# caoql98/LKGD

Measured on AMD Instinct MI355X. Metric: denoised frames/sec (14f x 576x1024, 25-step Euler), higher is better.
Workload: dtype f16; 1 GPU; SVD 14 frames x 576x1024, 25 Euler steps, CFG 1.0->3.0, single clip, vanilla pipeline_stable_video_diffusion_trans loop (configs[1]); unet=random-init SVD shapes (320,640,1280,1280), heads (5,10,20,20), 1.52 B params, parallelism=single GPU

## Files before the change

### lkgd_amd/csrc/gemm.hip

```cpp
#include "gemm_common.h"

#define BM 128
#define BN 128
#define STAGE_BYTES (2 * BM * BK * 2)
#define GEMM_LDS (2 * STAGE_BYTES)

__global__ __launch_bounds__(256, 2) void lkgd_gemm_kernel(const lkgd_gemm_desc p, int tiles_m, int tiles_n, int ksplit,
                                                           int per, float* ws) {
  extern __shared__ __attribute__((aligned(16))) char smem[];
  const int t = threadIdx.x;
  const int lane = t & 63;
  const int w = t >> 6;
  const int wr = w >> 1, wc = w & 1;

  const int nwg = tiles_m * tiles_n;
  const int bid = xcd_remap(blockIdx.x, nwg);
  const int tm = bid / tiles_n, tn = bid - tm * tiles_n;
  const int m0 = tm * BM, n0 = tn * BN;

  const int srow = t >> 3;
  const int schunk = (t & 7) ^ ((t >> 4) & 7);
  AGather<4> ag;
  const half_t* brow[4];
#pragma unroll
  for (int i = 0; i < 4; ++i) {
    ag.row[i] = a_row(p, m0 + srow + 32 * i);
    int n = n0 + srow + 32 * i;
    brow[i] = n < p.N ? (const half_t*)p.w + (long long)n * p.K + schunk * 8 : nullptr;
  }
  const int nk_all = p.K / BK;
  const int kb = ksplit > 1 ? (int)blockIdx.y * per : 0;
  const int ke = ksplit > 1 ? (kb + per < nk_all ? kb + per : nk_all) : nk_all;
  a_segment<4>(p, ag, kb * BK, schunk);

  auto stage = [&](int buf, int kt) {
    char* sa = smem + buf * STAGE_BYTES;
    char* sb = sa + BM * BK * 2;
    const int k0 = kt * BK;
    if (k0 >= ag.seg_end) a_segment<4>(p, ag, k0, schunk);
#pragma unroll
    for (int i = 0; i < 4; ++i) glds16(a_chunk<4>(ag, i, k0), sa + (w * 64 + 256 * i) * 16);
#pragma unroll
    for (int i = 0; i < 4; ++i)
      glds16(brow[i] ? brow[i] + k0 : (const half_t*)p.zeros, sb + (w * 64 + 256 * i) * 16);
  };

  float16_t acc[2][2];
#pragma unroll
  for (int i = 0; i < 2; ++i)
#pragma unroll
    for (int j = 0; j < 2; ++j)
#pragma unroll
      for (int r = 0; r < 16; ++r) acc[i][j][r] = 0.f;

  const int h = lane >> 5;
  int a_off[2], b_off[2], a_sw[2], b_sw[2];
#pragma unroll
  for (int i = 0; i < 2; ++i) {
    int ra = wr * 64 + i * 32 + (lane & 31);
    int rb = wc * 64 + i * 32 + (lane & 31);
    a_off[i] = ra * 128; a_sw[i] = (ra >> 1) & 7;
    b_off[i] = BM * BK * 2 + rb * 128; b_sw[i] = (rb >> 1) & 7;
  }

  stage(0, kb);
  asm volatile("s_waitcnt vmcnt(0)" ::: "memory");
  __syncthreads();
  for (int kt = kb; kt < ke; ++kt) {
    const int cur = (kt - kb) & 1;
    if (kt + 1 < ke) stage(cur ^ 1, kt + 1);
    const char* sbase = smem + cur * STAGE_BYTES;
#pragma unroll
    for (int ks = 0; ks < 4; ++ks) {
      half8_t af[2], bf[2];
#pragma unroll
      for (int i = 0; i < 2; ++i) {
        af[i] = *(const half8_t*)(sbase + a_off[i] + (((ks * 2 + h) ^ a_sw[i]) << 4));
        bf[i] = *(const half8_t*)(sbase + b_off[i] + (((ks * 2 + h) ^ b_sw[i]) << 4));
      }
#pragma unroll
      for (int i = 0; i < 2; ++i)
#pragma unroll
        for (int j = 0; j < 2; ++j)
          acc[i][j] = __builtin_amdgcn_mfma_f32_32x32x16_f16(af[i], bf[j], acc[i][j], 0, 0, 0);
    }
    asm volatile("s_waitcnt vmcnt(0)" ::: "memory");
    __syncthreads();
  }

  float* ct = (float*)smem;
#pragma unroll
  for (int i = 0; i < 2; ++i)
#pragma unroll
    for (int j = 0; j < 2; ++j)
#pragma unroll
      for (int r = 0; r < 16; ++r) {
        int row = wr * 64 + i * 32 + (r & 3) + 8 * (r >> 2) + 4 * h;
        int col = wc * 64 + j * 32 + (lane & 31);
        ct[row * BN + col] = acc[i][j][r];
      }
  __syncthreads();

  if (ksplit > 1) {
    float* dst = ws + (long long)blockIdx.y * p.M * p.N;
    const int col = (t & 31) * 4;
    if (n0 + col < p.N) {
      for (int row = t >> 5; row < BM && m0 + row < p.M; row += 8)
        *(float4_t*)(dst + (long long)(m0 + row) * p.N + n0 + col) = *(const float4_t*)(ct + row * BN + col);
    }
    return;
  }
  gemm_epilogue<BM, BN, 256>(p, ct, t, m0, n0, tn);
}

#define MID_NST 4
#define MID_NT 512
#define MID_LDS (MID_NST * STAGE_BYTES)
#define MID_LOADS 4

__global__ __launch_bounds__(MID_NT, 2) void lkgd_gemm_mid_kernel(const lkgd_gemm_desc p, int tiles_m, int tiles_n, int ksplit,
                                                                  int per, float* ws) {
  extern __shared__ __attribute__((aligned(16))) char smem[];
  const int t = threadIdx.x;
  const int lane = t & 63;
  const int w = t >> 6;
  const int wr = w >> 1, wc = w & 1;

  const int nwg = tiles_m * tiles_n;
  const int bid = xcd_remap(blockIdx.x, nwg);
  const int tm = bid / tiles_n, tn = bid - tm * tiles_n;
  const int m0 = tm * BM, n0 = tn * BN;

  const int srow = t >> 3;
  const int schunk = (t & 7) ^ ((t >> 4) & 7);
  AGather<2> ag;
  const half_t* brow[2];
#pragma unroll
  for (int i = 0; i < 2; ++i) {
    ag.row[i] = a_row(p, m0 + srow + 64 * i);
    int n = n0 + srow + 64 * i;
    brow[i] = n < p.N ? (const half_t*)p.w + (long long)n * p.K + schunk * 8 : nullptr;
  }
  const int nk_all = p.K / BK;
  const int kb = ksplit > 1 ? (int)blockIdx.y * per : 0;
  const int ke = ksplit > 1 ? (kb + per < nk_all ? kb + per : nk_all) : nk_all;
  const int nkt = ke - kb;
  a_segment<2>(p, ag, kb * BK, schunk);

  auto stage = [&](int buf, int kt) {
    char* sa = smem + buf * STAGE_BYTES;
    char* sb = sa + BM * BK * 2;
    const int k0 = kt * BK;
    if (k0 >= ag.seg_end) a_segment<2>(p, ag, k0, schunk);
#pragma unroll
    for (int i = 0; i < 2; ++i) glds16(a_chunk<2>(ag, i, k0), sa + (w * 64 + 512 * i) * 16);
#pragma unroll
    for (int i = 0; i < 2; ++i)
      glds16(brow[i] ? brow[i] + k0 : (const half_t*)p.zeros, sb + (w * 64 + 512 * i) * 16);
  };

  float16_t acc[2];
#pragma unroll
  for (int j = 0; j < 2; ++j)
#pragma unroll
    for (int r = 0; r < 16; ++r) acc[j][r] = 0.f;

  const int h = lane >> 5;
  const int ra = wr * 32 + (lane & 31);
  const int a_off = ra * 128, a_sw = (ra >> 1) & 7;
  int b_off[2], b_sw[2];
#pragma unroll
  for (int j = 0; j < 2; ++j) {
    int rb = wc * 64 + j * 32 + (lane & 31);
    b_off[j] = BM * BK * 2 + rb * 128; b_sw[j] = (rb >> 1) & 7;
  }

  for (int s = 0; s < MID_NST - 1 && s < nkt; ++s) stage(s, kb + s);
  int cur = 0;
  for (int i = 0; i < nkt; ++i) {
    const int newer = nkt - 1 - i;
#ifndef MID_X_NOBAR
    if (newer >= 2) asm volatile("s_waitcnt vmcnt(8)" ::: "memory");
    else if (newer == 1) asm volatile("s_waitcnt vmcnt(4)" ::: "memory");
    else asm volatile("s_waitcnt vmcnt(0)" ::: "memory");
    __builtin_amdgcn_s_barrier();
#endif
    const char* sbase = smem + cur * STAGE_BYTES;
    half8_t af[4], bf[4][2];
#pragma unroll
    for (int ks = 0; ks < 4; ++ks) {
#ifdef MID_X_NOLDS
      af[ks] = (half8_t)(half_t)(float)(lane + i);
#pragma unroll
      for (int j = 0; j < 2; ++j) bf[ks][j] = (half8_t)(half_t)(float)(lane - i + j);
#else
      af[ks] = *(const half8_t*)(sbase + a_off + (((ks * 2 + h) ^ a_sw) << 4));
#pragma unroll
      for (int j = 0; j < 2; ++j) bf[ks][j] = *(const half8_t*)(sbase + b_off[j] + (((ks * 2 + h) ^ b_sw[j]) << 4));
#endif
    }
#ifndef MID_X_NODMA
    if (i + MID_NST - 1 < nkt) {
      int nb = cur + MID_NST - 1; if (nb >= MID_NST) nb -= MID_NST;
      stage(nb, kb + i + MID_NST - 1);
    }
#endif
#pragma unroll
    for (int ks = 0; ks < 4; ++ks)
#pragma unroll
      for (int j = 0; j < 2; ++j) {
#ifdef MID_X_NOMFMA
        acc[j][ks] += (float)af[ks][j] * (float)bf[ks][j][0];
#else
        acc[j] = __builtin_amdgcn_mfma_f32_32x32x16_f16(af[ks], bf[ks][j], acc[j], 0, 0, 0);
#endif
      }
    cur = cur + 1 == MID_NST ? 0 : cur + 1;
  }
  __syncthreads();

  float* ct = (float*)smem;
#pragma unroll
  for (int j = 0; j < 2; ++j)
#pragma unroll
    for (int r = 0; r < 16; ++r) {
      int row = wr * 32 + (r & 3) + 8 * (r >> 2) + 4 * h;
      int col = wc * 64 + j * 32 + (lane & 31);
      ct[row * BN + col] = acc[j][r];
    }
  __syncthreads();

  if (ksplit > 1) {
    float* dst = ws + (long long)blockIdx.y * p.M * p.N;
    const int col = (t & 31) * 4;
    if (n0 + col < p.N) {
      for (int row = t >> 5; row < BM && m0 + row < p.M; row += 16)
        *(float4_t*)(dst + (long long)(m0 + row) * p.N + n0 + col) = *(const float4_t*)(ct + row * BN + col);
    }
    return;
  }
  gemm_epilogue<BM, BN, MID_NT>(p, ct, t, m0, n0, tn);
}

__global__ __launch_bounds__(256) void lkgd_gemm_splitk_reduce(const lkgd_gemm_desc p, int tiles_n, int ksplit,
                                                               const float* ws) {
  __shared__ __attribute__((aligned(16))) float ct[32 * BN];
  const int t = threadIdx.x;
  const int tm = blockIdx.x / tiles_n, tn = blockIdx.x - tm * tiles_n;
  const int m0 = tm * 32, n0 = tn * BN;
  const int col = (t & 31) * 4;
#pragma unroll
  for (int it = 0; it < 4; ++it) {
    const int row = (t >> 5) + 8 * it;
    float4_t v = {0.f, 0.f, 0.f, 0.f};
    if (m0 + row < p.M && n0 + col < p.N) {
      const float* src = ws + (long long)(m0 + row) * p.N + n0 + col;
      for (int s = 0; s < ksplit; ++s) v += *(const float4_t*)(src + (long long)s * p.M * p.N);
    }
    *(float4_t*)(ct + row * BN + col) = v;
  }
  __syncthreads();
  gemm_epilogue<32, BN, 256>(p, ct, t, m0, n0, tn);
}

#define BM2 256
#define NT2 512
#define STAGE2_BYTES ((BM2 + BN) * BK * 2)
#define NSTAGE2 3
#define GEMM2_LDS (NSTAGE2 * STAGE2_BYTES)

__global__ __launch_bounds__(NT2, 2) void lkgd_gemm_kernel_256(const lkgd_gemm_desc p, int tiles_m, int tiles_n) {
  extern __shared__ __attribute__((aligned(16))) char smem[];
  const int t = threadIdx.x;
  const int lane = t & 63;
  const int w = t >> 6;
  const int wr = w >> 1, wc = w & 1;
  const int nwg = tiles_m * tiles_n;
  const int bid = xcd_remap(blockIdx.x, nwg);
  const int tm = bid / tiles_n, tn = bid - tm * tiles_n;
  const int m0 = tm * BM2, n0 = tn * BN;

  const int srow = t >> 3;
  const int schunk = (t & 7) ^ ((t >> 4) & 7);
  AGather<4> ag;
  const half_t* brow[2];
#pragma unroll
  for (int i = 0; i < 4; ++i) ag.row[i] = a_row(p, m0 + srow + 64 * i);
  a_segment<4>(p, ag, 0, schunk);
#pragma unroll
  for (int i = 0; i < 2; ++i) {
    int n = n0 + srow + 64 * i;
    brow[i] = n < p.N ? (const half_t*)p.w + (long long)n * p.K + schunk * 8 : nullptr;
  }
  auto stage = [&](int buf, int kt) {
    char* sa = smem + buf * STAGE2_BYTES;
    char* sb = sa + BM2 * BK * 2;
    const int k0 = kt * BK;
    if (k0 >= ag.seg_end) a_segment<4>(p, ag, k0, schunk);
#pragma unroll
    for (int i = 0; i < 4; ++i) glds16(a_chunk<4>(ag, i, k0), sa + (w * 64 + 512 * i) * 16);
#pragma unroll
    for (int i = 0; i < 2; ++i)
      glds16(brow[i] ? brow[i] + k0 : (const half_t*)p.zeros, sb + (w * 64 + 512 * i) * 16);
  };

  float16_t acc[2][2];
#pragma unroll
  for (int i = 0; i < 2; ++i)
#pragma unroll
    for (int j = 0; j < 2; ++j)
#pragma unroll
      for (int r = 0; r < 16; ++r) acc[i][j][r] = 0.f;

  const int h = lane >> 5;
  int a_off[2], b_off[2], a_sw[2], b_sw[2];
#pragma unroll
  for (int i = 0; i < 2; ++i) {
    int ra = wr * 64 + i * 32 + (lane & 31);
    int rb = wc * 64 + i * 32 + (lane & 31);
    a_off[i] = ra * 128; a_sw[i] = (ra >> 1) & 7;
    b_off[i] = BM2 * BK * 2 + rb * 128; b_sw[i] = (rb >> 1) & 7;
  }

  const int nk = p.K / BK;
  stage(0, 0);
  if (nk > 1) stage(1, 1);
  int cur = 0;
  for (int kt = 0; kt < nk; ++kt) {
    if (kt + 1 < nk) asm volatile("s_waitcnt vmcnt(6)" ::: "memory");
    else asm volatile("s_waitcnt vmcnt(0)" ::: "memory");
    __builtin_amdgcn_s_barrier();
    if (kt + 2 < nk) {
      int nb = cur + 2; if (nb >= NSTAGE2) nb -= NSTAGE2;
      stage(nb, kt + 2);
    }
    const char* sbase = smem + cur * STAGE2_BYTES;
#pragma unroll
    for (int ks = 0; ks < 4; ++ks) {
      half8_t af[2], bf[2];
#pragma unroll
      for (int i = 0; i < 2; ++i) {
        af[i] = *(const half8_t*)(sbase + a_off[i] + (((ks * 2 + h) ^ a_sw[i]) << 4));
        bf[i] = *(const half8_t*)(sbase + b_off[i] + (((ks * 2 + h) ^ b_sw[i]) << 4));
      }
#pragma unroll
      for (int i = 0; i < 2; ++i)
#pragma unroll
        for (int j = 0; j < 2; ++j)
          acc[i][j] = __builtin_amdgcn_mfma_f32_32x32x16_f16(af[i], bf[j], acc[i][j], 0, 0, 0);
    }
    cur = cur + 1 == NSTAGE2 ? 0 : cur + 1;
  }
  __syncthreads();

  float* ct = (float*)smem;
#pragma unroll
  for (int i = 0; i < 2; ++i)
#pragma unroll
    for (int j = 0; j < 2; ++j)
#pragma unroll
      for (int r = 0; r < 16; ++r) {
        int row = wr * 64 + i * 32 + (r & 3) + 8 * (r >> 2) + 4 * h;
        int col = wc * 64 + j * 32 + (lane & 31);
        ct[row * BN + col] = acc[i][j][r];
      }
  __syncthreads();
  gemm_epilogue<BM2, BN, NT2>(p, ct, t, m0, n0, tn);
}


static int check_desc(const lkgd_gemm_desc* d) {
  if (!d || !d->a0 || !d->w || !d->out || !d->zeros) return LKGD_E_NULL;
  if (d->M <= 0 || d->N <= 0 || d->K <= 0) return LKGD_E_SHAPE;
  if (d->K % BK) return LKGD_E_SHAPE;
  if (d->N % 4) return LKGD_E_SHAPE;
  if (d->geglu != 0 && d->geglu != 32 && d->geglu != 80) return LKGD_E_MODE;
  if (d->geglu && (d->N % (4 * d->geglu) || d->rowbias || d->res1 || d->res2)) return LKGD_E_SHAPE;
  if (d->ldc % 4 || d->lda0 % 8) return LKGD_E_ALIGN;
  if (!aligned16(d->a0) || !aligned16(d->w) || !aligned16(d->zeros) || ((uintptr_t)d->out & 7)) return LKGD_E_ALIGN;
  if (d->a1 && (!aligned16(d->a1) || d->lda1 % 8)) return LKGD_E_ALIGN;
  if (d->bias && !aligned16(d->bias)) return LKGD_E_ALIGN;
  if (d->rowbias && (d->ldrb % 4 || d->rb_d1 <= 0 || d->rb_d2 <= 0 || d->rb_md <= 0 || d->rb_c0 < 0)) return LKGD_E_SHAPE;
  if (d->res1 && d->ldr1 % 4) return LKGD_E_ALIGN;
  if (d->res2 && d->ldr2 % 4) return LKGD_E_ALIGN;
  switch (d->mode) {
    case LKGD_A_PLAIN:
      if (d->csplit % 8 || d->csplit <= 0) return LKGD_E_SHAPE;
      if (d->csplit < d->K && !d->a1) return LKGD_E_NULL;
      if (d->csplit < d->K && d->csplit % BK) return LKGD_E_SHAPE;
      break;
    case LKGD_A_CONV3X3:
      if (d->Cin <= 0 || d->Cin % BK || d->K != 9 * d->Cin) return LKGD_E_SHAPE;
      if (d->csplit <= 0 || d->csplit % BK) return LKGD_E_SHAPE;
      if (d->csplit < d->Cin && !d->a1) return LKGD_E_NULL;
      if (d->Hout <= 0 || d->Wout <= 0 || d->Hin <= 0 || d->Win <= 0) return LKGD_E_SHAPE;
      if (d->stride != 1 && d->stride != 2) return LKGD_E_SHAPE;
      if (d->ups != 0 && d->ups != 1) return LKGD_E_SHAPE;
      if (d->M % (d->Hout * d->Wout)) return LKGD_E_SHAPE;
      if (d->pad_off != 0 && d->pad_off != 1) return LKGD_E_SHAPE;
      if (d->Hout != (((d->Hin << d->ups) - 1 - d->pad_off) / d->stride) + 1) return LKGD_E_SHAPE;
      if (d->Wout != (((d->Win << d->ups) - 1 - d->pad_off) / d->stride) + 1) return LKGD_E_SHAPE;
      break;
    case LKGD_A_TCONV3:
      if (d->Cin <= 0 || d->Cin % BK || d->K != 3 * d->Cin) return LKGD_E_SHAPE;
      if (d->F <= 0 || d->HW <= 0 || d->Floc <= 0 || d->f_off < 0 || d->f_off + d->Floc > d->F) return LKGD_E_SHAPE;
      if (d->M % (d->Floc * d->HW)) return LKGD_E_SHAPE;
      break;
    case LKGD_A_CONV3X3_C8:
      if (d->Cin != 8 || d->K != 128 || d->lda0 != 8 || d->stride != 1 || d->ups != 0 || d->pad_off != 0) return LKGD_E_SHAPE;
      if (d->Hout != d->Hin || d->Wout != d->Win || d->M % (d->Hout * d->Wout)) return LKGD_E_SHAPE;
      break;
    case LKGD_A_CCONV3:
      if (d->Cin <= 0 || d->Cin % BK || d->K != 27 * d->Cin || d->csplit != d->Cin) return LKGD_E_SHAPE;
      if (d->Hout <= 0 || d->Wout <= 0 || d->Hout != d->Hin || d->Wout != d->Win) return LKGD_E_SHAPE;
      if (d->stride != 1 || d->ups != 0 || d->pad_off != 0) return LKGD_E_SHAPE;
      if (d->Floc <= 0 || d->F != d->Floc + 2 || d->f_off != 0) return LKGD_E_SHAPE;
      if (d->M % (d->Floc * d->Hout * d->Wout)) return LKGD_E_SHAPE;
      if ((long long)(d->M / d->Floc) * d->F >= (1LL << 31)) return LKGD_E_SHAPE;
      if (d->geglu) return LKGD_E_SHAPE;
      break;
    default:
      return LKGD_E_MODE;
  }
  return LKGD_OK;
}

extern "C" int lkgd_gemm_stream_launch(const lkgd_gemm_desc* d, hipStream_t stream, int cus);
extern "C" int lkgd_gemm_wide_launch(const lkgd_gemm_desc* d, hipStream_t stream, int cus, int ksplit, int wn, int wm);
extern "C" int lkgd_gemm_wide_tile_n(int N);
extern "C" int lkgd_debug_wide_tile_n_forced();
extern "C" int lkgd_debug_wide_tile_m_forced();
extern "C" int lkgd_gemm_rowpanel_launch(const lkgd_gemm_desc* d, hipStream_t stream, int cus);
extern "C" int lkgd_gemm_resw_launch(const lkgd_gemm_desc* d, hipStream_t stream, int cus);
extern "C" int lkgd_gemm_resw_ok(const lkgd_gemm_desc* d, int cus);
extern "C" int lkgd_gemm_resw_colstats_ok(const lkgd_gemm_desc* d);

static thread_local int gemm_variant_override = 0;
extern "C" void lkgd_debug_set_gemm_variant(int v) { gemm_variant_override = (v >= 1 && v <= 7) ? v : 0; }
extern "C" void lkgd_debug_set_gemm_splitk(int on);

static thread_local bool gemm_splitk_enabled = true;
static thread_local int wide_ksplit_forced = 0;
extern "C" void lkgd_debug_set_wide_ksplit(int k) { wide_ksplit_forced = k < 0 ? 0 : k; }
static int wide_split(const lkgd_gemm_desc* d, long long tiles_wide, int cus) {
  if (d->geglu || !d->workspace || !aligned16(d->workspace)) return 0;
  const int nk = d->K / BK;
  if (wide_ksplit_forced) {
    const int c = wide_ksplit_forced;
    return (c >= 2 && nk % c == 0 && (long long)c * d->M * d->N * 4 <= d->workspace_bytes) ? c : 0;
  }
  if (!gemm_splitk_enabled || tiles_wide >= cus || nk < 48) return 0;
  const double unsplit = (double)tiles_wide / cus;
  int best = 0;
  double best_fill = 0.0;
  for (int c = 2; c <= 8 && c * 10 <= nk; ++c) {
    if (nk % c || (long long)c * d->M * d->N * 4 > d->workspace_bytes) continue;
    if (tiles_wide > 128 && c > 2) continue;
    const long long vt = tiles_wide * c, rounds = (vt + cus - 1) / cus;
    const double fill = (double)vt / (double)(rounds * cus);
    if (fill > best_fill + 1e-9) { best_fill = fill; best = c; }
  }
  return (best_fill >= 0.70 && best_fill >= unsplit + 0.15) ? best : 0;
}

extern "C" void lkgd_debug_set_gemm_splitk(int on) { gemm_splitk_enabled = on != 0; }

static thread_local float mid_tk_us = 0.75f, mid_fix_us = 6.0f, mid_red_us = 5.0f, mid_red_tbs = 3.5f;
static thread_local int mid_ksplit_forced = 0;
extern "C" void lkgd_debug_set_mid_model(float tk, float fix, float red, float tbs, int forced) {
  if (tk > 0) mid_tk_us = tk;
  if (fix > 0) mid_fix_us = fix;
  if (red > 0) mid_red_us = red;
  if (tbs > 0) mid_red_tbs = tbs;
  mid_ksplit_forced = forced < 0 ? 0 : forced;
}
static int mid_split(const lkgd_gemm_desc* d, long long nwg, int nk, int cus) {
  if (!d->workspace || !aligned16(d->workspace) || d->N % 4) return 1;
  const long long fit = d->workspace_bytes / ((long long)d->M * d->N * 4);
  if (mid_ksplit_forced) return (mid_ksplit_forced <= nk && mid_ksplit_forced <= fit) ? mid_ksplit_forced : 1;
  if (!gemm_splitk_enabled || nk < 16) return 1;
  int best = 1;
  float best_t = 1e30f;
  for (int ks = 1; ks <= 16 && ks <= fit && ks * 8 <= nk; ++ks) {
    const int per = (nk + ks - 1) / ks;
    const long long blocks = nwg * ((nk + per - 1) / per), rounds = (blocks + cus - 1) / cus;
    float t = (float)rounds * (mid_fix_us + per * mid_tk_us);
    if (ks > 1) t += mid_red_us + (float)ks * (float)d->M * (float)d->N * 4.0f / (mid_red_tbs * 1e6f);
    if (t < best_t * 0.97f) { best_t = t; best = ks; }
  }
  return best;
}

static int gemm_cus(int* cus_out) {
  static std::atomic<int> cus_of[64];
  int dev = 0;
  if (hipGetDevice(&dev) != hipSuccess || dev < 0 || dev > 63) return LKGD_E_LAUNCH;
  int cus = cus_of[dev].load(std::memory_order_relaxed);
  if (!cus) {
    hipDeviceProp_t prop;
    if (hipGetDeviceProperties(&prop, dev) != hipSuccess) return LKGD_E_LAUNCH;
    cus = prop.multiProcessorCount > 0 ? prop.multiProcessorCount : 256;
    cus_of[dev].store(cus, std::memory_order_relaxed);
  }
  *cus_out = cus;
  return LKGD_OK;
}

static int gemm_pick(const lkgd_gemm_desc* d, int cus, int* wide_ks_out) {
  const bool rows16 = d->N % 8 == 0 && d->ldc % 8 == 0 && aligned16(d->out) &&
                      (!d->res1 || (d->ldr1 % 8 == 0 && aligned16(d->res1))) &&
                      (!d->res2 || (d->ldr2 % 8 == 0 && aligned16(d->res2)));
  const int v = gemm_variant_override;
  const bool plain = d->mode == LKGD_A_PLAIN;
  const bool rp_ok = rows16 && plain && d->K <= 320 && d->csplit >= d->K && d->geglu != 80;
  const bool wide_ok = (d->geglu == 0 || (d->geglu == 80 && plain)) && d->mode != LKGD_A_CONV3X3_C8 &&
                       d->M < (1 << 24);
  const bool stream_ok = rows16 && d->geglu != 80;
  const bool rw_ok = lkgd_gemm_resw_ok(d, cus) != 0;
  const int wide_n = lkgd_gemm_wide_tile_n(d->N);
  const long long tiles_wide = (long long)((d->M + 255) / 256) * ((d->N + wide_n - 1) / wide_n);
  const bool n320 = d->N % wide_n == 0 || (long long)((d->N + 319) / 320) * 320 * 4 <= (long long)d->N * 5;
  int pick = 0;
  int wide_ks = 1;
  if (d->mode == LKGD_A_CCONV3) {
    if (!wide_ok || d->ln_colsum) return LKGD_E_SHAPE;
    *wide_ks_out = 1;
    return 4;
  }
  if (d->geglu == 80) {
    if (!wide_ok) return LKGD_E_SHAPE;
    pick = (rw_ok && (v == 6 || (v == 0 && d->M >= 32768))) ? 6 : 4;
  } else if (v != 0) {
    pick = v;
  } else if (rw_ok && d->res1 && d->M >= 32768) {
    pick = 6;
  } else if (rp_ok && d->M >= 4096 && d->K >= 192 && (d->res1 || (d->N != 320 && d->M >= 196608))) {
    pick = 5;
  } else if (wide_ok && d->geglu == 0 && d->N % 320 == 0 && d->M >= 1024 && (wide_ks = wide_split(d, tiles_wide, cus)) >= 2) {
    pick = 4;
  } else if (wide_ok && d->geglu == 0 && n320 && d->K >= 320 && tiles_wide * 2 >= cus - 16) {
    pick = 4;
  } else if (d->M < 12288) {
    wide_ks = 1;
    pick = (wide_ok && plain && d->geglu == 0 && d->N % 320 == 0 && d->N >= 2560 && d->M >= 2048 && !d->res1) ? 4 : 1;
    if (pick == 1 && d->geglu == 0 && (long long)((d->M + BM - 1) / BM) * ((d->N + BN - 1) / BN) <= cus) pick = 7;
  } else {
    pick = 3;
  }
  if (pick == 6 && !rw_ok) pick = d->geglu == 80 ? 4 : 1;
  if (pick == 5 && !rp_ok) pick = 1;
  if (d->ln_colsum) {
    if (!rp_ok || d->geglu || d->K % 64 || !aligned16(d->ln_colsum) || !(d->ln_eps > 0.f)) return LKGD_E_SHAPE;
    pick = 5;
  }
  if (pick == 4 && !wide_ok) pick = 3;
  if (pick == 3 && (!stream_ok || d->M <= 256)) pick = (d->K >= 960 && d->M > 256) ? 2 : 1;
  if (d->geglu == 80 && pick != 4 && pick != 6) return LKGD_E_SHAPE;
  *wide_ks_out = wide_ks;
  return pick;
}

static int gemm_wide_slices(const lkgd_gemm_desc* d, int cus, int pick, int wide_ks) {
  if (pick != 4) return 1;
  if (d->mode == LKGD_A_CCONV3) return 1;
  if (gemm_variant_override == 4) {
    const int wide_n = lkgd_gemm_wide_tile_n(d->N);
    const long long tiles_wide = (long long)((d->M + 255) / 256) * ((d->N + wide_n - 1) / wide_n);
    wide_ks = wide_n == 320 ? wide_split(d, tiles_wide, cus) : 1;
  }
  return wide_ks >= 2 ? wide_ks : 1;
}

static void gemm_wide_form(const lkgd_gemm_desc* d, int cus, int slices, int* wn_out, int* wm_out) {
  const int fn = lkgd_debug_wide_tile_n_forced(), fm = lkgd_debug_wide_tile_m_forced();
  int wn0 = lkgd_gemm_wide_tile_n(d->N);
  if (d->mode == LKGD_A_CCONV3 && d->N <= 256 && !fn) wn0 = 256;
  *wn_out = wn0;
  *wm_out = 256;
  if (slices != 1) return;
  if (fn || fm) {
    if (fm) *wm_out = fm;
    return;
  }
  const bool both = wn0 == 320 && d->mode == LKGD_A_PLAIN && !d->geglu && d->N % 320 == 0 && d->N % 256 == 0;
  float best = 0.f;
  for (int pass = 0; pass < 4; ++pass) {
    const int wm = (pass & 1) ? 192 : 256, wn = (pass & 2) ? 256 : wn0;
    if ((pass & 2) && !both) continue;
    if (pass && d->cs_rows > 0 && d->cs_rows % wm) continue;
    const long long tiles = (long long)((d->M + wm - 1) / wm) * ((d->N + wn - 1) / wn);
    const long long rounds = (tiles + cus - 1) / cus;
    const float unit = (wn == 256 ? 0.85f : 1.0f) * (wm == 192 ? (wn == 256 ? 0.72f / 0.85f : 0.83f) : 1.0f);
    const float cost = (float)rounds * unit;
    if (pass == 0) best = cost;
    else if (cost < best * 0.97f) { best = cost; *wn_out = wn; *wm_out = wm; }
  }
}

extern "C" int lkgd_gemm_wide_lds_out(const lkgd_gemm_desc* d, int ksplit, int wn);

static int tile128_split(const lkgd_gemm_desc* d, long long nwg, int cus, int* per_out) {
  int ksplit = 1, per = d->K / BK;
  const int nk = d->K / BK;
  const long long slots = 2LL * cus;
  if (gemm_splitk_enabled && d->workspace && aligned16(d->workspace) && d->N % 4 == 0 && nk >= 8 &&
      nwg * 10 < slots * 7) {
    const bool few = nwg * 2 <= slots;
    const int min_slice = few ? 4 : 32;
    long long cap = nk / min_slice;
    if (cap > 16) cap = 16;
    const long long fit = d->workspace_bytes / ((long long)d->M * d->N * 4);
    if (cap > fit) cap = fit;
    long long want = 1;
    for (long long ks = 2; ks <= cap; ++ks) {
      const long long blocks = nwg * ks, rounds = (blocks + slots - 1) / slots;
      if (blocks * 100 >= rounds * slots * 85 || (few && ks == cap)) { want = ks; break; }
    }
    if (few && slots / nwg > want && slots / nwg <= cap) want = slots / nwg;
    if (want >= 2) {
      per = (int)((nk + want - 1) / want);
      ksplit = (nk + per - 1) / per;
    }
  }
  *per_out = per;
  return ksplit;
}

struct gemm_plan {
  int pick;
  int ks, per;
  int wm, wn;
  int cs_blk;
  int lds_out;
};

static int gemm_make_plan(const lkgd_gemm_desc* d, int cus, gemm_plan* pl) {
  int wide_ks = 1;
  const int pick = gemm_pick(d, cus, &wide_ks);
  if (pick < 0) return pick;
  pl->pick = pick;
  pl->ks = 1;
  pl->per = d->K / BK;
  pl->wm = BM;
  pl->wn = BN;
  pl->cs_blk = 0;
  pl->lds_out = 0;
  const bool cs_shape = !d->geglu && d->N % 8 == 0;
  if (pick == 6) {
    pl->wm = 32; pl->wn = 160;
    if (cs_shape && lkgd_gemm_resw_colstats_ok(d)) pl->cs_blk = 32;
  } else if (pick == 5) {
    pl->wm = 256; pl->wn = 64;
  } else if (pick == 4) {
    pl->ks = gemm_wide_slices(d, cus, pick, wide_ks);
    gemm_wide_form(d, cus, pl->ks, &pl->wn, &pl->wm);
    pl->per = (d->K / BK) / pl->ks;
    if (cs_shape && pl->ks == 1 && d->ldc % 8 == 0 && aligned16(d->out) && d->N % pl->wn == 0) pl->cs_blk = pl->wm;
    const int lo = lkgd_gemm_wide_lds_out(d, pl->ks, pl->wn);
    pl->lds_out = lo > 0 ? 1 : 0;
  } else if (pick == 3 || pick == 2) {
    pl->wm = 256;
    if (pick == 2 && (long long)((d->M + BM2 - 1) / BM2) * ((d->N + BN - 1) / BN) > 0x7fffffffLL) return LKGD_E_SHAPE;
  } else {
    const long long nwg = (long long)((d->M + BM - 1) / BM) * ((d->N + BN - 1) / BN);
    if (nwg > 0x7fffffffLL) return LKGD_E_SHAPE;
    const int nk = d->K / BK;
    if (pick == 7) {
      const int ksplit = mid_split(d, nwg, nk, cus);
      if (ksplit > 1) {
        pl->per = (nk + ksplit - 1) / ksplit;
        pl->ks = (nk + pl->per - 1) / pl->per;
      }
    } else {
      pl->ks = tile128_split(d, nwg, cus, &pl->per);
    }
  }
  return LKGD_OK;
}

extern "C" int lkgd_gemm_plan(const lkgd_gemm_desc* d, int32_t cus, lkgd_gemm_plan_info* out) {
  if (!out) return LKGD_E_NULL;
  int rc = check_desc(d);
  if (rc != LKGD_OK) return rc;
  if (cus < 0) return LKGD_E_SHAPE;
  int n = cus;
  if (n == 0 && (rc = gemm_cus(&n)) != LKGD_OK) return rc;
  gemm_plan pl;
  if ((rc = gemm_make_plan(d, n, &pl)) != LKGD_OK) return rc;
  out->program = pl.pick;
  out->k_slices = pl.ks;
  out->tile_m = pl.wm;
  out->tile_n = pl.wn;
  out->colstats_block = pl.cs_blk;
  out->lds_out = pl.lds_out;
  return LKGD_OK;
}

extern "C" int lkgd_gemm_colstats_block(const lkgd_gemm_desc* d) {
  if (!d || check_desc(d) != LKGD_OK) return 0;
  int cus = 0;
  if (gemm_cus(&cus) != LKGD_OK) return 0;
  gemm_plan pl;
  return gemm_make_plan(d, cus, &pl) == LKGD_OK ? pl.cs_blk : 0;
}

extern "C" int lkgd_gemm_f16(const lkgd_gemm_desc* d, lkgd_stream_t stream) {
  int rc = check_desc(d);
  if (rc != LKGD_OK) return rc;
  LKGD_DEVICE_ONCE_BEGIN
    if (!lkgd_dynamic_lds(GEMM_LDS, lkgd_gemm_kernel) || !lkgd_dynamic_lds(GEMM2_LDS, lkgd_gemm_kernel_256) ||
        !lkgd_dynamic_lds(MID_LDS, lkgd_gemm_mid_kernel))
      return LKGD_E_LAUNCH;
  LKGD_DEVICE_ONCE_END
  int cus = 0;
  if ((rc = gemm_cus(&cus)) != LKGD_OK) return rc;
  gemm_plan pl;
  if ((rc = gemm_make_plan(d, cus, &pl)) != LKGD_OK) return rc;
  const int pick = pl.pick;
  if (d->colstats && pl.cs_blk == 0) return LKGD_E_SHAPE;
  if (pick == 6) return lkgd_gemm_resw_launch(d, (hipStream_t)stream, cus);
  if (pick == 5) return lkgd_gemm_rowpanel_launch(d, (hipStream_t)stream, cus);
  if (pick == 4) {
    const int ks = pl.ks;
    rc = lkgd_gemm_wide_launch(d, (hipStream_t)stream, cus, ks, pl.wn, pl.wm);
    if (rc != LKGD_OK || ks == 1) return rc;
    const int tn128 = (d->N + BN - 1) / BN;
    const unsigned rblocks = (unsigned)(((d->M + 31) / 32) * tn128);
    hipLaunchKernelGGL(lkgd_gemm_splitk_reduce, dim3(rblocks), dim3(256), 0, (hipStream_t)stream, *d, tn128, ks,
                       (const float*)d->workspace);
    return hipGetLastError() == hipSuccess ? LKGD_OK : LKGD_E_LAUNCH;
  }
  if (pick == 3) return lkgd_gemm_stream_launch(d, (hipStream_t)stream, cus);
  const int tiles_n = (d->N + BN - 1) / BN;
  if (pick == 2) {
    const int tiles_m = (d->M + BM2 - 1) / BM2;
    hipLaunchKernelGGL(lkgd_gemm_kernel_256, dim3((unsigned)(tiles_m * tiles_n)), dim3(NT2), GEMM2_LDS, (hipStream_t)stream, *d,
                       tiles_m, tiles_n);
    return hipGetLastError() == hipSuccess ? LKGD_OK : LKGD_E_LAUNCH;
  }
  const int tiles_m = (d->M + BM - 1) / BM;
  const unsigned nwg = (unsigned)(tiles_m * tiles_n);
  float* ws = pl.ks > 1 ? (float*)d->workspace : (float*)nullptr;
  const dim3 grid = pl.ks > 1 ? dim3(nwg, (unsigned)pl.ks) : dim3(nwg);
  if (pick == 7)
    hipLaunchKernelGGL(lkgd_gemm_mid_kernel, grid, dim3(MID_NT), MID_LDS, (hipStream_t)stream, *d, tiles_m, tiles_n, pl.ks, pl.per,
                       ws);
  else
    hipLaunchKernelGGL(lkgd_gemm_kernel, grid, dim3(256), GEMM_LDS, (hipStream_t)stream, *d, tiles_m, tiles_n, pl.ks, pl.per, ws);
  if (pl.ks > 1) {
    const unsigned rblocks = (unsigned)(((d->M + 31) / 32) * tiles_n);
    hipLaunchKernelGGL(lkgd_gemm_splitk_reduce, dim3(rblocks), dim3(256), 0, (hipStream_t)stream, *d, tiles_n, pl.ks,
                       (const float*)d->workspace);
  }
  return hipGetLastError() == hipSuccess ? LKGD_OK : LKGD_E_LAUNCH;
}
```

Before: 6.298 frames/s.

## Add dedicated thin-output 3x3 conv kernel for N<=8 channel convolutions

Adds a specialised implicit-GEMM kernel for 3x3 stride-1 convolutions with at most 8 output channels. The kernel keeps the whole weight tensor in LDS and stages an 8x16 spatial tile plus halo per 64-channel chunk with double buffering, then applies the nine taps through 16x16x32 MFMA. It replaces the generic 128-wide tiles, which waste most of their columns on such narrow outputs. The planner selects it automatically unless a variant override is set. The cost is extra LDS per block and a separate code path to maintain.

```diff
diff --git a/lkgd_amd/csrc/gemm.hip b/lkgd_amd/csrc/gemm.hip
--- a/lkgd_amd/csrc/gemm.hip
+++ b/lkgd_amd/csrc/gemm.hip
@@ -434,6 +434,8 @@
 extern "C" int lkgd_gemm_resw_launch(const lkgd_gemm_desc* d, hipStream_t stream, int cus);
 extern "C" int lkgd_gemm_resw_ok(const lkgd_gemm_desc* d, int cus);
 extern "C" int lkgd_gemm_resw_colstats_ok(const lkgd_gemm_desc* d);
+bool gemm_thin_conv_ok(const lkgd_gemm_desc* d);
+int gemm_thin_conv_launch(const lkgd_gemm_desc* d, hipStream_t stream);
 
 static thread_local int gemm_variant_override = 0;
 extern "C" void lkgd_debug_set_gemm_variant(int v) { gemm_variant_override = (v >= 1 && v <= 7) ? v : 0; }
@@ -632,7 +634,9 @@
   int wm, wn;
   int cs_blk;
   int lds_out;
+  int form;
 };
+enum { FORM_TILE = 0, FORM_THIN_CONV = 1 };
 
 static int gemm_make_plan(const lkgd_gemm_desc* d, int cus, gemm_plan* pl) {
   int wide_ks = 1;
@@ -645,6 +649,10 @@
   pl->wn = BN;
   pl->cs_blk = 0;
   pl->lds_out = 0;
+  pl->form = FORM_TILE;
+#ifndef GEMM_X_NO_SMALL_FORMS
+  if (gemm_variant_override == 0 && gemm_thin_conv_ok(d)) pl->form = FORM_THIN_CONV;
+#endif
   const bool cs_shape = !d->geglu && d->N % 8 == 0;
   if (pick == 6) {
     pl->wm = 32; pl->wn = 160;
@@ -718,6 +726,7 @@
   if ((rc = gemm_make_plan(d, cus, &pl)) != LKGD_OK) return rc;
   const int pick = pl.pick;
   if (d->colstats && pl.cs_blk == 0) return LKGD_E_SHAPE;
+  if (pl.form == FORM_THIN_CONV) return gemm_thin_conv_launch(d, (hipStream_t)stream);
   if (pick == 6) return lkgd_gemm_resw_launch(d, (hipStream_t)stream, cus);
   if (pick == 5) return lkgd_gemm_rowpanel_launch(d, (hipStream_t)stream, cus);
   if (pick == 4) {
diff --git a/lkgd_amd/csrc/gemm_small.hip b/lkgd_amd/csrc/gemm_small.hip
--- /dev/null
+++ b/lkgd_amd/csrc/gemm_small.hip
@@ -0,0 +1,121 @@
+#include "gemm_common.h"
+
+typedef float float4v_t __attribute__((ext_vector_type(4)));
+
+#define THIN_TH 8
+#define THIN_TW 16
+#define THIN_WP (THIN_TW + 2)
+#define THIN_NPIX ((THIN_TH + 2) * THIN_WP)
+#define THIN_NT 256
+#define THIN_LOADS 6
+#define THIN_STAGE (THIN_LOADS * THIN_NT * 16)
+#define THIN_W_MAX 65536
+
+__global__ __launch_bounds__(THIN_NT, 2) void lkgd_gemm_thin_conv_kernel(const lkgd_gemm_desc p, int tiles_y, int tiles_x) {
+  extern __shared__ __attribute__((aligned(16))) char smem[];
+  char* wl = smem + 2 * THIN_STAGE;
+  const int t = threadIdx.x;
+  const int lane = t & 63;
+  const int w = t >> 6;
+  const int per_img = tiles_y * tiles_x;
+  const int img = (int)blockIdx.x / per_img, rem = (int)blockIdx.x - img * per_img;
+  const int ty = rem / tiles_x, tx = rem - ty * tiles_x;
+  const int y0 = ty * THIN_TH, x0 = tx * THIN_TW;
+  const int H = p.Hout, W = p.Wout;
+  const int nc = p.Cin >> 6;
+
+  const half_t* src[THIN_LOADS];
+  unsigned ok = 0;
+#pragma unroll
+  for (int i = 0; i < THIN_LOADS; ++i) {
+    const int s = t + THIN_NT * i;
+    const int pp = s >> 3, lc = (s & 7) ^ (pp & 7);
+    const int py = pp / THIN_WP, px = pp - py * THIN_WP;
+    const int iy = y0 - 1 + py, ix = x0 - 1 + px;
+    const bool in = pp < THIN_NPIX && (unsigned)iy < (unsigned)H && (unsigned)ix < (unsigned)W;
+    const long long row = (long long)img * H * W + (long long)iy * W + ix;
+    src[i] = in ? (const half_t*)p.a0 + row * p.lda0 + lc * 8 : (const half_t*)p.zeros;
+    ok |= (in ? 1u : 0u) << i;
+  }
+  auto stage = [&](int buf, int c) {
+    char* sa = smem + buf * THIN_STAGE;
+#pragma unroll
+    for (int i = 0; i < THIN_LOADS; ++i)
+      glds16(src[i] + (((ok >> i) & 1u) ? c * 64 : 0), sa + (w * 64 + THIN_NT * i) * 16);
+  };
+  stage(0, 0);
+
+  {
+    const int chunks = p.N * (p.K >> 3);
+    for (int s = t; s < chunks; s += THIN_NT) *(half8_t*)(wl + (size_t)s * 16) = *(const half8_t*)((const half_t*)p.w + (size_t)s * 8);
+  }
+
+  const int col = lane & 15, kg = lane >> 4;
+  const bool bcol = col < p.N;
+  const char* wrow = wl + (size_t)(bcol ? col : 0) * p.K * 2 + kg * 16;
+  float4v_t acc[2];
+#pragma unroll
+  for (int g = 0; g < 2; ++g) acc[g] = (float4v_t){0.f, 0.f, 0.f, 0.f};
+  const half8_t z8 = {(half_t)0.f, (half_t)0.f, (half_t)0.f, (half_t)0.f, (half_t)0.f, (half_t)0.f, (half_t)0.f, (half_t)0.f};
+
+  asm volatile("s_waitcnt vmcnt(0)" ::: "memory");
+  __syncthreads();
+  for (int c = 0; c < nc; ++c) {
+    const int cur = c & 1;
+    if (c + 1 < nc) stage(cur ^ 1, c + 1);
+    const char* sa = smem + cur * THIN_STAGE;
+#pragma unroll
+    for (int ky = 0; ky < 3; ++ky) {
+      const char* wk = wrow + (size_t)((ky * nc + c) * 3) * 128;
+#pragma unroll
+      for (int kx = 0; kx < 3; ++kx) {
+#pragma unroll
+        for (int h = 0; h < 2; ++h) {
+          const half8_t bf = bcol ? *(const half8_t*)(wk + kx * 128 + h * 64) : z8;
+#pragma unroll
+          for (int g = 0; g < 2; ++g) {
+            const int pp = (2 * w + g + ky) * THIN_WP + col + kx;
+            const half8_t af = *(const half8_t*)(sa + pp * 128 + (((h * 4 + kg) ^ (pp & 7)) << 4));
+            acc[g] = __builtin_amdgcn_mfma_f32_16x16x32_f16(af, bf, acc[g], 0, 0, 0);
+          }
+        }
+      }
+    }
+    asm volatile("s_waitcnt vmcnt(0)" ::: "memory");
+    __syncthreads();
+  }
+
+  if (bcol) {
+    const float b = p.bias ? p.bias[col] : 0.f;
+#pragma unroll
+    for (int g = 0; g < 2; ++g) {
+      const int y = y0 + 2 * w + g;
+#pragma unroll
+      for (int i = 0; i < 4; ++i) {
+        const int x = x0 + 4 * kg + i;
+        if (y < H && x < W) {
+          const long long m = (long long)img * H * W + (long long)y * W + x;
+          ((half_t*)p.out)[m * p.ldc + col] = (half_t)((acc[g][i] + b) * p.s_acc);
+        }
+      }
+    }
+  }
+}
+
+__attribute__((visibility("hidden"))) bool gemm_thin_conv_ok(const lkgd_gemm_desc* d) {
+  return d->mode == LKGD_A_CONV3X3 && d->N <= 8 && d->stride == 1 && d->ups == 0 && d->pad_off == 0 && !d->a1 &&
+         d->Cin % 64 == 0 && !d->geglu && !d->ln_colsum && !d->colstats && !d->rowbias && !d->res1 && !d->res2 &&
+         d->M < (1 << 24) && (long long)d->N * d->K * 2 <= THIN_W_MAX;
+}
+
+__attribute__((visibility("hidden"))) int gemm_thin_conv_launch(const lkgd_gemm_desc* d, hipStream_t stream) {
+  LKGD_DEVICE_ONCE_BEGIN
+    if (!lkgd_dynamic_lds(2 * THIN_STAGE + THIN_W_MAX, lkgd_gemm_thin_conv_kernel)) return LKGD_E_LAUNCH;
+  LKGD_DEVICE_ONCE_END
+  const int tiles_y = (d->Hout + THIN_TH - 1) / THIN_TH, tiles_x = (d->Wout + THIN_TW - 1) / THIN_TW;
+  const long long grid = (long long)(d->M / (d->Hout * d->Wout)) * tiles_y * tiles_x;
+  if (grid > 0x7fffffffLL) return LKGD_E_SHAPE;
+  const size_t lds = 2 * THIN_STAGE + (size_t)d->N * d->K * 2;
+  hipLaunchKernelGGL(lkgd_gemm_thin_conv_kernel, dim3((unsigned)grid), dim3(THIN_NT), lds, stream, *d, tiles_y, tiles_x);
+  return hipGetLastError() == hipSuccess ? LKGD_OK : LKGD_E_LAUNCH;
+}
```

New measurement: 6.315 frames/s (median of 6 runs). Within noise of the previous version (+0.3%).
